# rainfall1998/3D_reconstruction_system

Hardware: AMD Instinct MI355X
Metric: Mpoints/s fused (1280x384 depth, N frames) (higher is better)
Workload: dtype f64; 1 GPU; C2: 1280x384 u8 depth x 100 frames per GPU -> float32 xyz, fused unproject+SE(3); every step reads the NEXT of 16 resident rasters (786 MB, beyond the 256 MiB Infinity Cache): fresh inputs from HBM, staged by the library's sweep, as in a pipeline that touches every frame once; inputs=fresh, frames_per_gpu=100, step=1 fused launch over this rank's frames (shards stay resident), assemble=none, assemble_choice=auto, parallelism=frames sharded, 1 rank(s), one process per GPU

## Files before the change

### 3d_reconstruction_system_amd/csrc/r3d_fuse.hip

```cpp
#include <algorithm>
#include <cstdlib>
#include <type_traits>

#include "r3d_internal.h"
#include "r3d_magic_div.h"
#include "r3d_voxel_dev.h"

namespace {

constexpr int kThreads = 256;
constexpr int kPx = 4;
constexpr int kTile = kThreads * kPx;
constexpr int kStageChunkMB = 96;

struct FuseDims {
  double scale;
  uint32_t hw;
  uint32_t width;
  uint32_t tiles_per_frame;
  uint32_t n_frames;
  uint32_t w_magic;
  uint32_t w_shift;
  uint32_t t_magic;
  uint32_t t_shift;
  uint32_t total_tiles;
  uint32_t rgb_vec_ok;
  uint32_t depth_vec_ok;
};

using r3d_magic::magic_div;
using r3d_magic::make_magic;

struct Pose {
  double r[9];
  double t[3];
};

template <bool POSE>
__device__ __forceinline__ void load_pose(const double* __restrict__ pose, uint32_t frame, Pose& P) {
  if (POSE) {
    const double* pp = pose + (uint64_t)frame * 12;
#pragma unroll
    for (int k = 0; k < 9; ++k) P.r[k] = pp[k];
#pragma unroll
    for (int k = 0; k < 3; ++k) P.t[k] = pp[9 + k];
  }
}

template <bool POSE>
__device__ __forceinline__ void point(double z, double u, double v, const Pose& p, double o[3]) {
  const double x = u * z;
  const double y = v * z;
  if (POSE) {
    const double dx = x - p.t[0], dy = y - p.t[1], dz = z - p.t[2];
    o[0] = fma(p.r[2], dz, fma(p.r[1], dy, p.r[0] * dx));
    o[1] = fma(p.r[5], dz, fma(p.r[4], dy, p.r[3] * dx));
    o[2] = fma(p.r[8], dz, fma(p.r[7], dy, p.r[6] * dx));
  } else {
    o[0] = x;
    o[1] = y;
    o[2] = z;
  }
}

typedef float f32x3 __attribute__((ext_vector_type(3)));
typedef uint32_t u32x4 __attribute__((ext_vector_type(4)));
typedef uint32_t u32x3 __attribute__((ext_vector_type(3)));

__device__ __forceinline__ void store_x3_nt(void* dst, f32x3 v) {
  asm volatile("global_store_dwordx3 %0, %1, off nt\n\ts_nop 1" ::"v"(dst), "v"(v) : "memory");
}
__device__ __forceinline__ void store_x3_nt(void* dst, u32x3 v) {
  asm volatile("global_store_dwordx3 %0, %1, off nt\n\ts_nop 1" ::"v"(dst), "v"(v) : "memory");
}

template <typename DT, int ITEMS, int SHIFT, bool CLAMP>
__device__ __forceinline__ void load_tile(const DT* __restrict__ depth, const FuseDims& dm, uint32_t tile, uint32_t tid,
                                          DT raw[ITEMS]) {
  const uint32_t frame = magic_div(tile, dm.t_magic, dm.t_shift);
  const uint32_t tf = tile - frame * dm.tiles_per_frame;
  const uint64_t fbase = (uint64_t)frame * dm.hw;
#pragma unroll
  for (int r = 0; r < ITEMS; ++r) {
    const uint32_t p = tf * kTile + ((r * kThreads + tid) >> SHIFT);
    if (CLAMP)
      raw[r] = depth[fbase + min(p, dm.hw - 1)];
    else
      raw[r] = p < dm.hw ? depth[fbase + p] : DT(0);
  }
}

template <int ROUNDS>
__device__ __forceinline__ void load_tile_wave(const uint8_t* __restrict__ depth, const FuseDims& dm, uint64_t fbase, uint32_t tf,
                                               uint32_t tid, uint8_t raw[ROUNDS]) {
  const uint32_t lane = tid & 63u, wave = tid >> 6;
  const bool whole = dm.depth_vec_ok && (tf + 1) * kTile <= dm.hw;
  if (whole) {
    const uint32_t dw = reinterpret_cast<const uint32_t*>(depth + fbase + (uint64_t)tf * kTile)[tid];
#pragma unroll
    for (int r = 0; r < ROUNDS; ++r) {
      const uint32_t got = (uint32_t)__builtin_amdgcn_ds_bpermute((int)((16u * r + (lane >> 2)) << 2), (int)dw);
      raw[r] = (uint8_t)(got >> (8u * (lane & 3u)));
    }
  } else {
#pragma unroll
    for (int r = 0; r < ROUNDS; ++r) {
      const uint32_t p = tf * kTile + 256u * wave + 64u * r + lane;
      raw[r] = depth[fbase + min(p, dm.hw - 1)];
    }
  }
}

struct StageSlices {
  const uint4* src;
  uint64_t n16;
  uint32_t n_stage;
};

__device__ __forceinline__ uint32_t touch_pieces(const uint4* __restrict__ src, uint64_t lo, uint64_t hi) {
  uint32_t acc = 0;
  for (uint64_t base = lo + threadIdx.x; base < hi; base += kThreads * 4) {
    uint4 q[4];
#pragma unroll
    for (int k = 0; k < 4; ++k) {
      const uint64_t i = base + (uint64_t)k * kThreads;
      q[k] = src[i < hi ? i : hi - 1];
    }
#pragma unroll
    for (int k = 0; k < 4; ++k) acc ^= q[k].x ^ q[k].y ^ q[k].z ^ q[k].w;
  }
  return acc;
}

template <bool POSE, bool RAGGED>
__device__ __forceinline__ void store_tile(float* __restrict__ out, const FuseDims& dm, const Pose& P, uint64_t fbase,
                                           const uint32_t p[kPx], const double z[kPx], const double ui[kPx],
                                           const double vj[kPx]) {
#pragma unroll
  for (int r = 0; r < kPx; ++r) {
    double w[3];
    point<POSE>(z[r], ui[r], vj[r], P, w);
    if (!RAGGED || p[r] < dm.hw) store_x3_nt(out + (fbase + p[r]) * 3, f32x3{(float)w[0], (float)w[1], (float)w[2]});
  }
}

template <typename DT, bool POSE, bool WAVE>
__global__ __launch_bounds__(kThreads) void fuse_lane_kernel(const DT* __restrict__ depth, float* __restrict__ out,
                                                             const double* __restrict__ u, const double* __restrict__ v,
                                                             const double* __restrict__ pose, const FuseDims dm,
                                                             const StageSlices st) {
  if (blockIdx.x < st.n_stage) {
    const uint64_t lo = st.n16 * blockIdx.x / st.n_stage, hi = st.n16 * (blockIdx.x + 1) / st.n_stage;
    const uint32_t acc = touch_pieces(st.src, lo, hi);
    if (acc == 0x9e3779b9u && st.n16 == ~(uint64_t)0) out[0] = (float)acc;
    return;
  }
  const uint32_t tid = threadIdx.x;
  const uint32_t first = WAVE ? 256u * (tid >> 6) + (tid & 63u) : tid;
  constexpr uint32_t kRound = WAVE ? 64u : (uint32_t)kThreads;
  for (uint32_t tile = blockIdx.x - st.n_stage; tile < dm.total_tiles; tile += gridDim.x - st.n_stage) {
    const uint32_t frame = magic_div(tile, dm.t_magic, dm.t_shift);
    const uint32_t tf = tile - frame * dm.tiles_per_frame;
    Pose P;
    load_pose<POSE>(pose, frame, P);
    const uint64_t fbase = (uint64_t)frame * dm.hw;
    const uint32_t t0 = tf * kTile;
    DT raw[kPx];
    if constexpr (WAVE)
      load_tile_wave<kPx>(depth, dm, fbase, tf, tid, raw);
    else
      load_tile<DT, kPx, 0, true>(depth, dm, tile, tid, raw);
    uint32_t p[kPx];
    double z[kPx], ui[kPx], vj[kPx];
#pragma unroll
    for (int r = 0; r < kPx; ++r) {
      p[r] = t0 + r * kRound + first;
      const uint32_t pc = min(p[r], dm.hw - 1);
      const uint32_t j = magic_div(pc, dm.w_magic, dm.w_shift);
      ui[r] = u[pc - j * dm.width];
      vj[r] = v[j];
    }
    __builtin_amdgcn_s_waitcnt(0);
#pragma unroll
    for (int r = 0; r < kPx; ++r) z[r] = (double)raw[r] * dm.scale;
    if (t0 + kTile <= dm.hw)
      store_tile<POSE, false>(out, dm, P, fbase, p, z, ui, vj);
    else
      store_tile<POSE, true>(out, dm, P, fbase, p, z, ui, vj);
  }
}

template <typename DT, bool POSE>
__global__ __launch_bounds__(kThreads) void fuse_pair_kernel(const DT* __restrict__ depth, double* __restrict__ out,
                                                             const double* __restrict__ u, const double* __restrict__ v,
                                                             const double* __restrict__ pose, const FuseDims dm) {
  constexpr int kItems = 2 * kPx;
  const uint32_t tid = threadIdx.x;
  const bool odd = tid & 1u;
  for (uint32_t tile = blockIdx.x; tile < dm.total_tiles; tile += gridDim.x) {
    const uint32_t frame = magic_div(tile, dm.t_magic, dm.t_shift);
    const uint32_t tf = tile - frame * dm.tiles_per_frame;
    Pose P;
    load_pose<POSE>(pose, frame, P);
    double ra[3], rb[3];
    if (POSE) {
#pragma unroll
      for (int c = 0; c < 3; ++c) {
        ra[c] = odd ? P.r[3 + c] : P.r[c];
        rb[c] = odd ? P.r[6 + c] : P.r[3 + c];
      }
    }
    const uint64_t fbase = (uint64_t)frame * dm.hw;
    DT raw[kItems];
    load_tile<DT, kItems, 1, (sizeof(DT) > 1)>(depth, dm, tile, tid, raw);
    uint32_t* tile_out = reinterpret_cast<uint32_t*>(out) + (fbase + (uint64_t)tf * kTile) * 6;
#pragma unroll
    for (int r = 0; r < kItems; ++r) {
      const uint32_t q = r * kThreads + tid;
      const uint32_t p = tf * kTile + (q >> 1);
      if (p < dm.hw) {
        const uint32_t j = magic_div(p, dm.w_magic, dm.w_shift);
        const uint32_t i = p - j * dm.width;
        const double z = (double)raw[r] * dm.scale;
        const double x = u[i] * z;
        const double y = v[j] * z;
        double a, b;
        if (POSE) {
          const double dx = x - P.t[0], dy = y - P.t[1], dz = z - P.t[2];
          a = fma(ra[2], dz, fma(ra[1], dy, ra[0] * dx));
          b = fma(rb[2], dz, fma(rb[1], dy, rb[0] * dx));
        } else {
          a = odd ? y : x;
          b = odd ? z : y;
        }
        const uint32_t alo = (uint32_t)__double2loint(a), ahi = (uint32_t)__double2hiint(a);
        const uint32_t blo = (uint32_t)__double2loint(b), bhi = (uint32_t)__double2hiint(b);
        store_x3_nt(tile_out + (uint64_t)q * 3, odd ? u32x3{ahi, blo, bhi} : u32x3{alo, ahi, blo});
      }
    }
  }
}

template <typename DT, bool POSE>
__global__ __launch_bounds__(kThreads) void fuse_rgb_kernel(const DT* __restrict__ depth, const uint8_t* __restrict__ rgb,
                                                            float* __restrict__ out, uint32_t* __restrict__ rgba_out,
                                                            const double* __restrict__ u, const double* __restrict__ v,
                                                            const double* __restrict__ pose, const FuseDims dm) {
  __shared__ __attribute__((aligned(16))) uint8_t lds[kTile * 3];
  const uint32_t tid = threadIdx.x;
  auto is_staged = [&](uint32_t tile) {
    const uint32_t frame = magic_div(tile, dm.t_magic, dm.t_shift);
    const uint32_t tf = tile - frame * dm.tiles_per_frame;
    return dm.rgb_vec_ok && (tf + 1) * kTile <= dm.hw;
  };
  auto colour_chunk = [&](uint32_t tile) -> u32x4 {
    const uint32_t frame = magic_div(tile, dm.t_magic, dm.t_shift);
    const uint32_t tf = tile - frame * dm.tiles_per_frame;
    return reinterpret_cast<const u32x4*>(rgb + ((uint64_t)frame * dm.hw + (uint64_t)tf * kTile) * 3)[tid];
  };
  for (uint32_t tile = blockIdx.x; tile < dm.total_tiles; tile += gridDim.x) {
    const uint32_t frame = magic_div(tile, dm.t_magic, dm.t_shift);
    const uint32_t tf = tile - frame * dm.tiles_per_frame;
    Pose P;
    load_pose<POSE>(pose, frame, P);
    const uint64_t fbase = (uint64_t)frame * dm.hw;
    const bool staged = is_staged(tile);
    DT raw[kPx];
    u32x4 ccur = {0, 0, 0, 0};
    load_tile<DT, kPx, 0, true>(depth, dm, tile, tid, raw);
    if (staged && tid < kTile * 3 / 16) ccur = colour_chunk(tile);
    if (staged) {
      if (tid < kTile * 3 / 16) reinterpret_cast<u32x4*>(lds)[tid] = ccur;
      __syncthreads();
    }
#pragma unroll
    for (int r = 0; r < kPx; ++r) {
      const uint32_t l = r * kThreads + tid;
      const uint32_t p = tf * kTile + l;
      if (p < dm.hw) {
        const uint32_t j = magic_div(p, dm.w_magic, dm.w_shift);
        const uint32_t i = p - j * dm.width;
        double w[3];
        point<POSE>((double)raw[r] * dm.scale, u[i], v[j], P, w);
        store_x3_nt(out + (fbase + p) * 3, f32x3{(float)w[0], (float)w[1], (float)w[2]});
        uint32_t c;
        if (staged) {
          c = (uint32_t)lds[l * 3] | ((uint32_t)lds[l * 3 + 1] << 8) | ((uint32_t)lds[l * 3 + 2] << 16);
        } else {
          const uint8_t* s = rgb + (fbase + p) * 3;
          c = (uint32_t)s[0] | ((uint32_t)s[1] << 8) | ((uint32_t)s[2] << 16);
        }
        __builtin_nontemporal_store(c, rgba_out + fbase + p);
      }
    }
    if (staged) __syncthreads();
  }
}

constexpr uint64_t kVoxelRun = 64;

struct VoxelView {
  uint64_t* table;
  unsigned long long* counters;
  double factor;
  int log2cap;
};

template <typename DT, bool POSE, bool RGB>
__global__ __launch_bounds__(kThreads) void fuse_voxel_kernel(const DT* __restrict__ depth, const uint8_t* __restrict__ rgb,
                                                              float* __restrict__ out, uint32_t* __restrict__ rgba_out,
                                                              const double* __restrict__ u, const double* __restrict__ v,
                                                              const double* __restrict__ pose, const FuseDims dm,
                                                              const VoxelView vv) {
  using namespace r3d_vox;
  __shared__ __attribute__((aligned(16))) uint8_t lds[RGB ? kTile * 3 : 16];
  __shared__ unsigned long long local_set[kLdsSlots];
  __shared__ unsigned local_fill[3];
  const uint32_t tid = threadIdx.x;
  const int lane = tid & 63;
  const uint64_t mask = ((uint64_t)1 << vv.log2cap) - 1;
  unsigned n_new = 0, n_ignored = 0, n_over = 0;
  const uint32_t per_wg = (dm.total_tiles + gridDim.x - 1) / gridDim.x;
  const uint64_t lo64 = (uint64_t)blockIdx.x * per_wg;
  const uint32_t tile_lo = lo64 < dm.total_tiles ? (uint32_t)lo64 : dm.total_tiles;
  const uint32_t tile_hi = dm.total_tiles - tile_lo < per_wg ? dm.total_tiles : tile_lo + per_wg;
  for (int k = tid; k < kLdsSlots; k += kThreads) local_set[k] = kEmpty;
  if (tid < 3) local_fill[tid] = 0;
  auto flush = [&]() {
#pragma unroll
    for (int k = 0; k < kLdsSlots / kThreads; ++k) {
      const int s = k * kThreads + tid;
      const uint64_t code = local_set[s];
      if (code != kEmpty) {
        local_set[s] = kEmpty;
        const int r = table_insert(vv.table, mask, vv.log2cap, code);
        n_new += r > 0 ? 1u : 0u;
        n_over += r < 0 ? 1u : 0u;
      }
    }
  };
  unsigned total = 0, j = 0;
  for (uint32_t tile = tile_lo; tile < tile_hi; ++tile, ++j) {
    lds_settle();
    __syncthreads();
    if (j > 0) total += local_fill[(j - 1) % 3];
    if (tid == 0) local_fill[(j + 1) % 3] = 0;
    if (total >= (unsigned)kLdsKeepBelow) {
      flush();
      total = 0;
    }
    const uint32_t frame = magic_div(tile, dm.t_magic, dm.t_shift);
    const uint32_t tf = tile - frame * dm.tiles_per_frame;
    Pose P;
    load_pose<POSE>(pose, frame, P);
    const uint64_t fbase = (uint64_t)frame * dm.hw;
    const bool staged = RGB && dm.rgb_vec_ok && (tf + 1) * kTile <= dm.hw;
    DT raw[kPx];
    load_tile<DT, kPx, 0, true>(depth, dm, tile, tid, raw);
    if (RGB && staged && tid < kTile * 3 / 16)
      reinterpret_cast<u32x4*>(lds)[tid] = reinterpret_cast<const u32x4*>(rgb + (fbase + (uint64_t)tf * kTile) * 3)[tid];
    lds_settle();
    __syncthreads();
    unsigned claimed = 0;
#pragma unroll
    for (int r = 0; r < kPx; ++r) {
      const uint32_t l = r * kThreads + tid;
      const uint32_t p = tf * kTile + l;
      uint64_t code = kEmpty;
      bool live = p < dm.hw;
      if (live) {
        const uint32_t jrow = magic_div(p, dm.w_magic, dm.w_shift);
        const uint32_t i = p - jrow * dm.width;
        double w[3];
        point<POSE>((double)raw[r] * dm.scale, u[i], v[jrow], P, w);
        const float fx = (float)w[0], fy = (float)w[1], fz = (float)w[2];
        store_x3_nt(out + (fbase + p) * 3, f32x3{fx, fy, fz});
        if (RGB) {
          uint32_t c;
          if (staged) {
            c = (uint32_t)lds[l * 3] | ((uint32_t)lds[l * 3 + 1] << 8) | ((uint32_t)lds[l * 3 + 2] << 16);
          } else {
            const uint8_t* sp = rgb + (fbase + p) * 3;
            c = (uint32_t)sp[0] | ((uint32_t)sp[1] << 8) | ((uint32_t)sp[2] << 16);
          }
          __builtin_nontemporal_store(c, rgba_out + fbase + p);
        }
        if (!voxel_key(fx, fy, fz, vv.factor, &code)) {
          ++n_ignored;
          live = false;
          code = kEmpty;
        }
      }
      const uint64_t prev = prev_lane_u64(code);
      if (live && lane > 0 && prev == code) live = false;
      if (live) {
        bool mine = false;
        const bool done = lds_set_claim(local_set, code, &mine);
        claimed += mine ? 1u : 0u;
        if (!done) {
          const int r2 = table_insert(vv.table, mask, vv.log2cap, code);
          n_new += r2 > 0 ? 1u : 0u;
          n_over += r2 < 0 ? 1u : 0u;
        }
      }
    }
#pragma unroll
    for (int off = 32; off > 0; off >>= 1) claimed += __shfl_down(claimed, off, 64);
    if (lane == 0 && claimed) atomicAdd(&local_fill[j % 3], claimed);
  }
  __syncthreads();
  flush();
  const auto [w_new, w_ignored, w_over] = r3d_vox::wave_sum(n_new, n_ignored, n_over);
  if (lane == 0) {
    if (w_new) atomicAdd(&vv.counters[0], (unsigned long long)w_new);
    if (w_ignored) atomicAdd(&vv.counters[1], (unsigned long long)w_ignored);
    if (w_over) atomicAdd(&vv.counters[2], (unsigned long long)w_over);
  }
}

__global__ __launch_bounds__(kThreads) void rgb_expand_kernel(const uint8_t* __restrict__ rgb, uint32_t* __restrict__ rgba_out,
                                                              uint64_t n, uint32_t vec_ok) {
  __shared__ __attribute__((aligned(16))) uint8_t lds[kTile * 3];
  const uint32_t tid = threadIdx.x;
  const uint64_t n_tiles = (n + kTile - 1) / kTile;
  for (uint64_t tile = blockIdx.x; tile < n_tiles; tile += gridDim.x) {
    const uint64_t base = tile * kTile;
    const bool staged = vec_ok && base + kTile <= n;
    if (staged) {
      if (tid < kTile * 3 / 16) reinterpret_cast<uint4*>(lds)[tid] = reinterpret_cast<const uint4*>(rgb + base * 3)[tid];
      __syncthreads();
    }
#pragma unroll
    for (int r = 0; r < kPx; ++r) {
      const uint32_t l = r * kThreads + tid;
      if (base + l < n) {
        uint32_t c;
        if (staged) {
          c = (uint32_t)lds[l * 3] | ((uint32_t)lds[l * 3 + 1] << 8) | ((uint32_t)lds[l * 3 + 2] << 16);
        } else {
          const uint8_t* s = rgb + (base + l) * 3;
          c = (uint32_t)s[0] | ((uint32_t)s[1] << 8) | ((uint32_t)s[2] << 16);
        }
        __builtin_nontemporal_store(c, rgba_out + base + l);
      }
    }
    if (staged) __syncthreads();
  }
}

__global__ __launch_bounds__(kThreads) void cache_touch_kernel(const uint4* __restrict__ src, uint64_t n16,
                                                               uint32_t* __restrict__ sink) {
  uint32_t acc = 0;
  const uint64_t stride = (uint64_t)gridDim.x * (kThreads * 4);
  for (uint64_t base = (uint64_t)blockIdx.x * (kThreads * 4) + threadIdx.x; base < n16; base += stride) {
    uint4 q[4];
#pragma unroll
    for (int k = 0; k < 4; ++k) {
      const uint64_t i = base + (uint64_t)k * kThreads;
      q[k] = src[i < n16 ? i : n16 - 1];
    }
#pragma unroll
    for (int k = 0; k < 4; ++k) acc ^= q[k].x ^ q[k].y ^ q[k].z ^ q[k].w;
  }
  if (acc == 0x9e3779b9u && n16 == ~(uint64_t)0) *sink = acc;
}

StageSlices stage_slices(const r3d_ctx* ctx, const void* p, uint64_t bytes) {
  const uintptr_t lo = ((uintptr_t)p + 15) & ~(uintptr_t)15, hi = ((uintptr_t)p + bytes) & ~(uintptr_t)15;
  if (hi <= lo) return StageSlices{nullptr, 0, 0};
  const uint64_t n16 = (hi - lo) / 16;
  uint64_t blocks = (n16 + kThreads * 4 - 1) / (kThreads * 4);
  if (blocks > (uint64_t)ctx->num_cus * 8) blocks = (uint64_t)ctx->num_cus * 8;
  return StageSlices{reinterpret_cast<const uint4*>(lo), n16, (uint32_t)blocks};
}

void cache_touch(r3d_ctx* ctx, const void* p, uint64_t bytes) {
  const StageSlices st = stage_slices(ctx, p, bytes);
  if (!st.n_stage) return;
  hipLaunchKernelGGL(cache_touch_kernel, dim3(st.n_stage), dim3(kThreads), 0, ctx->stream, st.src, st.n16,
                     static_cast<uint32_t*>(nullptr));
}

struct FusePtrs {
  const void* depth;
  void* out;
  const double* u;
  const double* v;
  const double* pose;
  const uint8_t* rgb;
  uint32_t* rgba;
};

template <typename DT, bool POSE>
void launch_typed(const FusePtrs& p, const FuseDims& dm, int out_dtype, int blocks, bool wave, const StageSlices& st,
                  hipStream_t s) {
  const DT* d = static_cast<const DT*>(p.depth);
  if (out_dtype == R3D_F64) {
    hipLaunchKernelGGL((fuse_pair_kernel<DT, POSE>), dim3(blocks), dim3(kThreads), 0, s, d, static_cast<double*>(p.out), p.u,
                       p.v, p.pose, dm);
  } else if (p.rgb) {
    hipLaunchKernelGGL((fuse_rgb_kernel<DT, POSE>), dim3(blocks), dim3(kThreads), 0, s, d, p.rgb, static_cast<float*>(p.out),
                       p.rgba, p.u, p.v, p.pose, dm);
  } else {
    if constexpr (std::is_same<DT, uint8_t>::value && !POSE) {
      if (wave) {
        hipLaunchKernelGGL((fuse_lane_kernel<DT, POSE, true>), dim3(blocks + st.n_stage), dim3(kThreads), 0, s, d,
                           static_cast<float*>(p.out), p.u, p.v, p.pose, dm, st);
        return;
      }
    }
    hipLaunchKernelGGL((fuse_lane_kernel<DT, POSE, false>), dim3(blocks + st.n_stage), dim3(kThreads), 0, s, d,
                       static_cast<float*>(p.out), p.u, p.v, p.pose, dm, st);
  }
}

template <bool POSE>
void launch_depth(const FusePtrs& p, const FuseDims& dm, int depth_dtype, int out_dtype, int blocks, bool wave,
                  const StageSlices& st, hipStream_t s) {
  switch (depth_dtype) {
    case R3D_DEPTH_U8: launch_typed<uint8_t, POSE>(p, dm, out_dtype, blocks, wave, st, s); break;
    case R3D_DEPTH_U16: launch_typed<uint16_t, POSE>(p, dm, out_dtype, blocks, wave, st, s); break;
    default: launch_typed<float, POSE>(p, dm, out_dtype, blocks, wave, st, s); break;
  }
}

template <typename DT>
void launch_voxel_typed(const FusePtrs& p, const FuseDims& dm, const VoxelView& vv, bool with_pose, int blocks, hipStream_t s) {
  const DT* d = static_cast<const DT*>(p.depth);
  float* o = static_cast<float*>(p.out);
#define R3D_LAUNCH_FV(POSE, RGB)                                                                                         \
  hipLaunchKernelGGL((fuse_voxel_kernel<DT, POSE, RGB>), dim3(blocks), dim3(kThreads), 0, s, d, p.rgb, o, p.rgba, p.u, p.v, \
                     p.pose, dm, vv)
  if (with_pose) {
    if (p.rgb) R3D_LAUNCH_FV(true, true); else R3D_LAUNCH_FV(true, false);
  } else {
    if (p.rgb) R3D_LAUNCH_FV(false, true); else R3D_LAUNCH_FV(false, false);
  }
#undef R3D_LAUNCH_FV
}

void launch_voxel(const FusePtrs& p, const FuseDims& dm, const VoxelView& vv, int depth_dtype, bool with_pose, int blocks,
                  hipStream_t s) {
  switch (depth_dtype) {
    case R3D_DEPTH_U8: launch_voxel_typed<uint8_t>(p, dm, vv, with_pose, blocks, s); break;
    case R3D_DEPTH_U16: launch_voxel_typed<uint16_t>(p, dm, vv, with_pose, blocks, s); break;
    default: launch_voxel_typed<float>(p, dm, vv, with_pose, blocks, s); break;
  }
}

int fuse_common(r3d_ctx* ctx, const r3d_camera* cam, const void* d_depth, int depth_dtype, int n_frames,
                double depth_scale, const double* d_pose, bool with_pose, void* d_out, int out_dtype,
                const uint8_t* d_rgb = nullptr, uint32_t* d_rgba = nullptr, r3d_voxelset* vs = nullptr) {
  int rc = r3d_ctx_enter(ctx);
  if (rc) return rc;
  R3D_REQUIRE(cam != nullptr, "camera is NULL");
  VoxelView vv{nullptr, nullptr, 0.0, 0};
  if (vs) {
    r3d_ctx* vctx = nullptr;
    if ((rc = r3d_voxelset_device_view(vs, &vctx, &vv.factor, &vv.table, &vv.log2cap, &vv.counters))) return rc;
    R3D_REQUIRE(vctx == ctx, "voxel set belongs to a different ctx");
    R3D_REQUIRE(out_dtype == R3D_F32, "the voxel keys are taken from the f32 cloud: out_dtype must be R3D_F32");
  }
  R3D_REQUIRE(cam->ctx == ctx, "camera belongs to a different ctx");
  R3D_REQUIRE(depth_dtype >= R3D_DEPTH_U8 && depth_dtype <= R3D_DEPTH_F32, "unknown depth dtype %d", depth_dtype);
  R3D_REQUIRE(out_dtype == R3D_F32 || out_dtype == R3D_F64, "unknown output dtype %d", out_dtype);
  R3D_REQUIRE(n_frames >= 0, "n_frames must be >= 0");
  R3D_REQUIRE((d_rgb == nullptr) == (d_rgba == nullptr), "colour needs both the rgb plane and the rgba output");
  if (n_frames == 0) return R3D_OK;
  R3D_REQUIRE(d_depth && d_out, "NULL device pointer");
  R3D_REQUIRE(!with_pose || d_pose, "pose table is NULL");
  const uint64_t hw = (uint64_t)cam->height * cam->width;
  const uint64_t dsz = r3d_depth_size(depth_dtype), osz = 3 * (uint64_t)r3d_xyz_size(out_dtype);
  {
    const uint64_t all_tiles = ((hw + kTile - 1) / kTile) * (uint64_t)n_frames;
    R3D_REQUIRE(all_tiles < ((uint64_t)1 << 31), "batch too large for one launch (%llu tiles); split the frames",
                (unsigned long long)all_tiles);
  }
  const bool colour_after = d_rgb && out_dtype == R3D_F64;
  const bool wave = !with_pose && out_dtype == R3D_F32 && depth_dtype == R3D_DEPTH_U8 && !(d_rgb && !colour_after);
  const bool rgb_in_kernel = d_rgb && !colour_after;
  const uint64_t in_per_frame = hw * (dsz + (rgb_in_kernel ? 3 : 0));
  const uint64_t in_bytes = in_per_frame * (uint64_t)n_frames;
  const uint64_t chunk_bytes = (uint64_t)(ctx->fuse_chunk_mb > 0 ? ctx->fuse_chunk_mb : kStageChunkMB) << 20;
  const uint64_t budget = (uint64_t)ctx->fuse_resident_mb << 20;
  const uint64_t depth_bytes = hw * dsz * (uint64_t)n_frames, rgb_bytes = rgb_in_kernel ? hw * 3 * (uint64_t)n_frames : 0;
  const bool small_inputs = dsz <= 2 || (out_dtype == R3D_F64 && !rgb_in_kernel);
  bool stage_depth = ctx->fuse_prefetch == 2, stage_rgb = ctx->fuse_prefetch == 2 && rgb_in_kernel;
  if (ctx->fuse_prefetch == 0 && small_inputs && in_bytes > ((uint64_t)ctx->fuse_stage_auto_mb << 20)) {
    stage_depth = !r3d_inputs_resident(ctx, d_depth, depth_bytes, budget);
    stage_rgb = rgb_in_kernel && !r3d_inputs_resident(ctx, d_rgb, rgb_bytes, budget);
  }
  const bool stage = stage_depth || stage_rgb;
  r3d_wrote(ctx, d_out, hw * osz * (uint64_t)n_frames);
  r3d_inputs_read(ctx, d_depth, depth_bytes, budget);
  if (rgb_in_kernel) r3d_inputs_read(ctx, d_rgb, rgb_bytes, budget);
  int frames_per_step = n_frames;
  if (stage) {
    const uint64_t f = chunk_bytes / (in_per_frame ? in_per_frame : 1);
    frames_per_step = (int)(f < 1 ? 1 : (f > (uint64_t)n_frames ? (uint64_t)n_frames : f));
  }
  for (int f0 = 0; f0 < n_frames; f0 += frames_per_step) {
    const int nf = n_frames - f0 < frames_per_step ? n_frames - f0 : frames_per_step;
    const uint64_t px0 = hw * (uint64_t)f0;
    const char* dd = static_cast<const char*>(d_depth) + px0 * dsz;
    const uint8_t* rr = d_rgb ? d_rgb + px0 * 3 : nullptr;
    FusePtrs p{dd, static_cast<char*>(d_out) + px0 * osz, cam->d_u, cam->d_v, with_pose ? d_pose + (uint64_t)f0 * 12 : nullptr,
               colour_after ? nullptr : rr, d_rgba ? d_rgba + px0 : nullptr};
    FuseDims dm;
    dm.scale = depth_scale;
    dm.hw = (uint32_t)hw;
    dm.width = (uint32_t)cam->width;
    dm.tiles_per_frame = (uint32_t)((hw + kTile - 1) / kTile);
    dm.n_frames = (uint32_t)nf;
    make_magic(dm.width, &dm.w_magic, &dm.w_shift);
    make_magic(dm.tiles_per_frame, &dm.t_magic, &dm.t_shift);
    const uint64_t total_tiles = (uint64_t)dm.tiles_per_frame * nf;
    dm.total_tiles = (uint32_t)total_tiles;
    dm.rgb_vec_ok = rr && ((uintptr_t)rr % 16 == 0) && (hw % 16 == 0);
    dm.depth_vec_ok = ((uintptr_t)dd % 4 == 0) && ((hw * dsz) % 4 == 0);
    const bool fold = stage_depth && ctx->fuse_stage_fold && !vs && out_dtype == R3D_F32 && !p.rgb && total_tiles < (1u << 30);
    StageSlices st{nullptr, 0, 0};
    if (fold)
      st = stage_slices(ctx, dd, hw * dsz * (uint64_t)nf);
    else if (stage_depth)
      cache_touch(ctx, dd, hw * dsz * (uint64_t)nf);
    if (stage_rgb) cache_touch(ctx, rr, hw * 3 * (uint64_t)nf);
    ctx->fuse_sweeps += (int)stage_depth + (int)stage_rgb;
    const bool stride8 = !wave && !with_pose && out_dtype == R3D_F32 && depth_dtype == R3D_DEPTH_U8 && !p.rgb;
    uint64_t blocks = ctx->fuse_blocks > 0 ? (uint64_t)ctx->fuse_blocks : stride8 ? (uint64_t)ctx->num_cus * 8 : total_tiles;
    if (blocks > total_tiles) blocks = total_tiles;
    if (vs) {
      uint64_t g = ctx->fuse_blocks > 0 ? (uint64_t)ctx->fuse_blocks
                                         : std::max<uint64_t>((uint64_t)ctx->num_cus * 8, (total_tiles + kVoxelRun - 1) / kVoxelRun);
      if (g > total_tiles) g = total_tiles;
      launch_voxel(p, dm, vv, depth_dtype, with_pose, (int)g, ctx->stream);
    } else if (with_pose)
      launch_depth<true>(p, dm, depth_dtype, out_dtype, (int)blocks, wave, st, ctx->stream);
    else
      launch_depth<false>(p, dm, depth_dtype, out_dtype, (int)blocks, wave, st, ctx->stream);
  }
  if (colour_after) {
    const uint64_t n = hw * (uint64_t)n_frames;
    uint64_t b = (n + kTile - 1) / kTile;
    if (b > (uint64_t)ctx->num_cus * 16) b = (uint64_t)ctx->num_cus * 16;
    hipLaunchKernelGGL(rgb_expand_kernel, dim3((unsigned)b), dim3(kThreads), 0, ctx->stream, d_rgb, d_rgba, n,
                       (uint32_t)((uintptr_t)d_rgb % 16 == 0));
  }
  R3D_HIP(hipGetLastError());
  return R3D_OK;
}

int fuse_host_common(r3d_ctx* ctx, const r3d_camera* cam, const void* h_depth, int depth_dtype, int n_frames,
                     double depth_scale, const double* h_pose, bool with_pose, void* h_out, int out_dtype) {
  int rc = r3d_ctx_enter(ctx);
  if (rc) return rc;
  R3D_REQUIRE(cam != nullptr, "camera is NULL");
  R3D_REQUIRE(depth_dtype >= R3D_DEPTH_U8 && depth_dtype <= R3D_DEPTH_F32, "unknown depth dtype %d", depth_dtype);
  R3D_REQUIRE(out_dtype == R3D_F32 || out_dtype == R3D_F64, "unknown output dtype %d", out_dtype);
  R3D_REQUIRE(n_frames >= 0, "n_frames must be >= 0");
  if (n_frames == 0) return R3D_OK;
  R3D_REQUIRE(h_depth && h_out, "NULL host pointer");
  R3D_REQUIRE(!with_pose || h_pose, "pose table is NULL");
  const size_t n = (size_t)cam->height * cam->width * n_frames;
  const size_t in_bytes = n * r3d_depth_size(depth_dtype);
  const size_t out_bytes = n * 3 * r3d_xyz_size(out_dtype);
  void *d_in = nullptr, *d_out = nullptr, *d_pose = nullptr;
  if ((rc = r3d_scratch(ctx, 0, in_bytes, &d_in))) return rc;
  if ((rc = r3d_scratch(ctx, 1, out_bytes, &d_out))) return rc;
  if (with_pose) {
    if ((rc = r3d_scratch(ctx, 2, (size_t)n_frames * 12 * sizeof(double), &d_pose))) return rc;
    R3D_HIP(hipMemcpyAsync(d_pose, h_pose, (size_t)n_frames * 12 * sizeof(double), hipMemcpyHostToDevice, ctx->stream));
  }
  const size_t frame_in = (size_t)cam->height * cam->width * r3d_depth_size(depth_dtype);
  const size_t frame_out = (size_t)cam->height * cam->width * 3 * r3d_xyz_size(out_dtype);
  auto launch = [&](int64_t lo, int64_t n) -> int {
    return fuse_common(ctx, cam, static_cast<char*>(d_in) + (size_t)lo * frame_in, depth_dtype, (int)n, depth_scale,
                       with_pose ? static_cast<const double*>(d_pose) + (size_t)lo * 12 : nullptr, with_pose,
                       static_cast<char*>(d_out) + (size_t)lo * frame_out, out_dtype);
  };
  return r3d_host_pipeline(ctx, n_frames, frame_in, frame_out, h_depth, h_out, d_in, d_out, launch);
}

int fuse_rgb_host(r3d_ctx* ctx, const r3d_camera* cam, const void* h_depth, int depth_dtype, int n_frames, double depth_scale,
                  const double* h_pose, const unsigned char* h_rgb, void* h_xyz_out, int out_dtype, uint32_t* h_rgba_out) {
  int rc = r3d_ctx_enter(ctx);
  if (rc) return rc;
  R3D_REQUIRE(cam != nullptr, "camera is NULL");
  R3D_REQUIRE(depth_dtype >= R3D_DEPTH_U8 && depth_dtype <= R3D_DEPTH_F32, "unknown depth dtype %d", depth_dtype);
  R3D_REQUIRE(out_dtype == R3D_F32 || out_dtype == R3D_F64, "unknown output dtype %d", out_dtype);
  R3D_REQUIRE(n_frames >= 0, "n_frames must be >= 0");
  if (n_frames == 0) return R3D_OK;
  R3D_REQUIRE(h_depth && h_rgb && h_xyz_out && h_rgba_out, "NULL host pointer");
  const size_t px = (size_t)cam->height * cam->width, n = px * n_frames;
  const size_t f_depth = px * r3d_depth_size(depth_dtype), f_rgb = px * 3, f_xyz = px * 3 * r3d_xyz_size(out_dtype),
               f_rgba = px * 4;
  void *d_depth = nullptr, *d_xyz = nullptr, *d_pose = nullptr, *d_rgb = nullptr, *d_rgba = nullptr;
  if ((rc = r3d_scratch(ctx, 0, n * r3d_depth_size(depth_dtype), &d_depth))) return rc;
  if ((rc = r3d_scratch(ctx, 1, n * 3 * r3d_xyz_size(out_dtype), &d_xyz))) return rc;
  if ((rc = r3d_scratch(ctx, 3, n * 3, &d_rgb))) return rc;
  if ((rc = r3d_scratch(ctx, 4, n * 4, &d_rgba))) return rc;
  if (h_pose) {
    if ((rc = r3d_scratch(ctx, 2, (size_t)n_frames * 12 * sizeof(double), &d_pose))) return rc;
    R3D_HIP(hipMemcpyAsync(d_pose, h_pose, (size_t)n_frames * 12 * sizeof(double), hipMemcpyHostToDevice, ctx->stream));
  }
  const r3d_pipe_buf ins[2] = {{const_cast<void*>(h_depth), d_depth, f_depth}, {const_cast<unsigned char*>(h_rgb), d_rgb, f_rgb}};
  const r3d_pipe_buf outs[2] = {{h_xyz_out, d_xyz, f_xyz}, {h_rgba_out, d_rgba, f_rgba}};
  auto launch = [&](int64_t lo, int64_t cnt) -> int {
    return fuse_common(ctx, cam, static_cast<char*>(d_depth) + (size_t)lo * f_depth, depth_dtype, (int)cnt, depth_scale,
                       h_pose ? static_cast<const double*>(d_pose) + (size_t)lo * 12 : nullptr, h_pose != nullptr,
                       static_cast<char*>(d_xyz) + (size_t)lo * f_xyz, out_dtype,
                       static_cast<const uint8_t*>(d_rgb) + (size_t)lo * f_rgb, static_cast<uint32_t*>(d_rgba) + (size_t)lo * px);
  };
  return r3d_host_pipeline_multi(ctx, n_frames, ins, 2, outs, 2, launch);
}

}

extern "C" {

int r3d_selftest_magic_div(uint32_t d, uint32_t x, uint32_t* q_out) {
  if (d == 0 || x >= ((uint32_t)1 << 31) || !q_out) {
    r3d_set_error("r3d_selftest_magic_div: d must be >= 1, x < 2^31");
    return R3D_ERR_INVALID;
  }
  uint32_t m = 0, sh = 0;
  make_magic(d, &m, &sh);
  *q_out = (uint32_t)(((uint64_t)x * m) >> sh);
  return R3D_OK;
}

int r3d_cache_prefetch(r3d_ctx* ctx, const void* d_ptr, size_t bytes) {
  int rc = r3d_ctx_enter(ctx);
  if (rc) return rc;
  if (bytes == 0) return R3D_OK;
  R3D_REQUIRE(d_ptr != nullptr, "NULL device pointer");
  cache_touch(ctx, d_ptr, bytes);
  r3d_inputs_read(ctx, d_ptr, bytes, (size_t)ctx->fuse_resident_mb << 20);
  R3D_HIP(hipGetLastError());
  return R3D_OK;
}

int r3d_unproject(r3d_ctx* ctx, const r3d_camera* cam, const void* d_depth, int depth_dtype, int n_frames,
                  double depth_scale, void* d_xyz_out, int out_dtype) {
  return fuse_common(ctx, cam, d_depth, depth_dtype, n_frames, depth_scale, nullptr, false, d_xyz_out, out_dtype);
}

int r3d_unproject_host(r3d_ctx* ctx, const r3d_camera* cam, const void* h_depth, int depth_dtype, int n_frames,
                       double depth_scale, void* h_xyz_out, int out_dtype) {
  return fuse_host_common(ctx, cam, h_depth, depth_dtype, n_frames, depth_scale, nullptr, false, h_xyz_out,
                          out_dtype);
}

int r3d_fuse_frames(r3d_ctx* ctx, const r3d_camera* cam, const void* d_depth, int depth_dtype, int n_frames,
                    double depth_scale, const double* d_pose, void* d_xyz_out, int out_dtype) {
  return fuse_common(ctx, cam, d_depth, depth_dtype, n_frames, depth_scale, d_pose, true, d_xyz_out, out_dtype);
}

int r3d_fuse_frames_host(r3d_ctx* ctx, const r3d_camera* cam, const void* h_depth, int depth_dtype, int n_frames,
                         double depth_scale, const double* h_pose, void* h_xyz_out, int out_dtype) {
  return fuse_host_common(ctx, cam, h_depth, depth_dtype, n_frames, depth_scale, h_pose, true, h_xyz_out,
                          out_dtype);
}

int r3d_fuse_frames_rgb(r3d_ctx* ctx, const r3d_camera* cam, const void* d_depth, int depth_dtype, int n_frames,
                        double depth_scale, const double* d_pose, const unsigned char* d_rgb, void* d_xyz_out,
                        int out_dtype, uint32_t* d_rgba_out) {
  R3D_REQUIRE(n_frames == 0 || (d_rgb && d_rgba_out), "colour plane / rgba output is NULL");
  return fuse_common(ctx, cam, d_depth, depth_dtype, n_frames, depth_scale, d_pose, d_pose != nullptr, d_xyz_out, out_dtype,
                     d_rgb, d_rgba_out);
}

int r3d_fuse_frames_voxel(r3d_ctx* ctx, const r3d_camera* cam, const void* d_depth, int depth_dtype, int n_frames,
                          double depth_scale, const double* d_pose, const unsigned char* d_rgb, float* d_xyz_out,
                          uint32_t* d_rgba_out, r3d_voxelset* vs) {
  R3D_REQUIRE(vs != nullptr, "voxel set is NULL");
  R3D_REQUIRE((d_rgb == nullptr) == (d_rgba_out == nullptr), "colour needs both the rgb plane and the rgba output");
  R3D_REQUIRE(ctx != nullptr && cam != nullptr, "NULL argument");
  {
    r3d_ctx* vctx = nullptr;
    VoxelView view;
    int rc = r3d_voxelset_device_view(vs, &vctx, &view.factor, &view.table, &view.log2cap, &view.counters);
    if (rc) return rc;
    R3D_REQUIRE(vctx == ctx, "voxel set belongs to a different ctx");
  }
  const bool with_pose = d_pose != nullptr;
  const int64_t hw = (int64_t)cam->height * cam->width, total = hw * (int64_t)n_frames;
  const int path = ctx->voxel_path;
  if (path == 1 || n_frames <= 0 || !r3d_voxelset_sort_feasible(vs, total, path == 2)) {
    if (n_frames > 0) ctx->voxel_last_path = 1;
    return fuse_common(ctx, cam, d_depth, depth_dtype, n_frames, depth_scale, d_pose, with_pose, d_xyz_out, R3D_F32, d_rgb,
                       d_rgba_out, vs);
  }
  const int64_t want = (int64_t)1 << 18;
  const int f0 = path == 2 ? n_frames : (int)std::min<int64_t>(n_frames, std::max<int64_t>(1, (want + hw - 1) / hw));
  int rc = fuse_common(ctx, cam, d_depth, depth_dtype, f0, depth_scale, d_pose, with_pose, d_xyz_out, R3D_F32, d_rgb, d_rgba_out);
  if (rc) return rc;
  bool sort = path == 2;
  if (!sort && (rc = r3d_voxelset_sample(vs, d_xyz_out, hw * f0, total, 1.5, &sort))) return rc;
  const size_t dsz = r3d_depth_size(depth_dtype);
  const char* depth_rest = static_cast<const char*>(d_depth) + (size_t)hw * f0 * dsz;
  const double* pose_rest = with_pose ? d_pose + (size_t)f0 * 12 : nullptr;
  const unsigned char* rgb_rest = d_rgb ? d_rgb + (size_t)hw * f0 * 3 : nullptr;
  uint32_t* rgba_rest = d_rgba_out ? d_rgba_out + (size_t)hw * f0 : nullptr;
  float* xyz_rest = d_xyz_out + (size_t)hw * f0 * 3;
  if (sort) {
    if (f0 < n_frames && (rc = fuse_common(ctx, cam, depth_rest, depth_dtype, n_frames - f0, depth_scale, pose_rest, with_pose, xyz_rest,
                                           R3D_F32, rgb_rest, rgba_rest)))
      return rc;
    return r3d_voxelset_insert_path(vs, d_xyz_out, total, 2);
  }
  if ((rc = r3d_voxelset_insert_path(vs, d_xyz_out, hw * f0, 1))) return rc;
  if (f0 == n_frames) return R3D_OK;
  return fuse_common(ctx, cam, depth_rest, depth_dtype, n_frames - f0, depth_scale, pose_rest, with_pose, xyz_rest, R3D_F32, rgb_rest,
                     rgba_rest, vs);
}

int r3d_fuse_frames_rgb_host(r3d_ctx* ctx, const r3d_camera* cam, const void* h_depth, int depth_dtype, int n_frames,
                             double depth_scale, const double* h_pose, const unsigned char* h_rgb, void* h_xyz_out,
                             int out_dtype, uint32_t* h_rgba_out) {
  return fuse_rgb_host(ctx, cam, h_depth, depth_dtype, n_frames, depth_scale, h_pose, h_rgb, h_xyz_out, out_dtype, h_rgba_out);
}

}
```

Before: 506,800 Mpoints/s.

## Fold cache staging sweep into f64, RGB and voxel fuse kernels

Extends the in-kernel staging prologue, where extra leading workgroups touch the depth/colour input, from the f32 depth kernel to the f64 pair, RGB and voxel kernels. This replaces a separate cache_touch launch, and a new helper splits a capped staging-workgroup budget between the depth and colour sweeps. The f64 pair kernel also gets an occupancy hint in its launch bounds. This removes a launch and serialisation, but staging blocks now compete with the fuse blocks for bandwidth and CUs.

Result: no change. 507,000 Mpoints/s, median of 3 (+0.0%).

```diff
diff --git a/3d_reconstruction_system_amd/csrc/r3d_fuse.hip b/3d_reconstruction_system_amd/csrc/r3d_fuse.hip
--- a/3d_reconstruction_system_amd/csrc/r3d_fuse.hip
+++ b/3d_reconstruction_system_amd/csrc/r3d_fuse.hip
@@ -132,6 +132,26 @@
   return acc;
 }
 
+__device__ __forceinline__ void stage_slice(const StageSlices& st, uint32_t wg, void* sink) {
+  const uint64_t lo = st.n16 * wg / st.n_stage, hi = st.n16 * (wg + 1) / st.n_stage;
+  const uint32_t acc = touch_pieces(st.src, lo, hi);
+  if (acc == 0x9e3779b9u && st.n16 == ~(uint64_t)0) *static_cast<uint32_t*>(sink) = acc;
+}
+
+__device__ __forceinline__ bool stage_prologue(const StageSlices& st, void* sink) {
+  if (blockIdx.x >= st.n_stage) return false;
+  stage_slice(st, blockIdx.x, sink);
+  return true;
+}
+
+__device__ __forceinline__ bool stage_prologue(const StageSlices& sd, const StageSlices& sc, void* sink) {
+  if (blockIdx.x >= sd.n_stage + sc.n_stage) return false;
+  const bool first = blockIdx.x < sd.n_stage;
+  const StageSlices st{first ? sd.src : sc.src, first ? sd.n16 : sc.n16, first ? sd.n_stage : sc.n_stage};
+  stage_slice(st, first ? blockIdx.x : blockIdx.x - sd.n_stage, sink);
+  return true;
+}
+
 template <bool POSE, bool RAGGED>
 __device__ __forceinline__ void store_tile(float* __restrict__ out, const FuseDims& dm, const Pose& P, uint64_t fbase,
                                            const uint32_t p[kPx], const double z[kPx], const double ui[kPx],
@@ -149,12 +169,7 @@
                                                              const double* __restrict__ u, const double* __restrict__ v,
                                                              const double* __restrict__ pose, const FuseDims dm,
                                                              const StageSlices st) {
-  if (blockIdx.x < st.n_stage) {
-    const uint64_t lo = st.n16 * blockIdx.x / st.n_stage, hi = st.n16 * (blockIdx.x + 1) / st.n_stage;
-    const uint32_t acc = touch_pieces(st.src, lo, hi);
-    if (acc == 0x9e3779b9u && st.n16 == ~(uint64_t)0) out[0] = (float)acc;
-    return;
-  }
+  if (stage_prologue(st, out)) return;
   const uint32_t tid = threadIdx.x;
   const uint32_t first = WAVE ? 256u * (tid >> 6) + (tid & 63u) : tid;
   constexpr uint32_t kRound = WAVE ? 64u : (uint32_t)kThreads;
@@ -191,13 +206,15 @@
 }
 
 template <typename DT, bool POSE>
-__global__ __launch_bounds__(kThreads) void fuse_pair_kernel(const DT* __restrict__ depth, double* __restrict__ out,
+__global__ __launch_bounds__(kThreads, 8) void fuse_pair_kernel(const DT* __restrict__ depth, double* __restrict__ out,
                                                              const double* __restrict__ u, const double* __restrict__ v,
-                                                             const double* __restrict__ pose, const FuseDims dm) {
+                                                             const double* __restrict__ pose, const FuseDims dm,
+                                                             const StageSlices st) {
+  if (stage_prologue(st, out)) return;
   constexpr int kItems = 2 * kPx;
   const uint32_t tid = threadIdx.x;
   const bool odd = tid & 1u;
-  for (uint32_t tile = blockIdx.x; tile < dm.total_tiles; tile += gridDim.x) {
+  for (uint32_t tile = blockIdx.x - st.n_stage; tile < dm.total_tiles; tile += gridDim.x - st.n_stage) {
     const uint32_t frame = magic_div(tile, dm.t_magic, dm.t_shift);
     const uint32_t tf = tile - frame * dm.tiles_per_frame;
     Pose P;
@@ -245,8 +262,11 @@
 __global__ __launch_bounds__(kThreads) void fuse_rgb_kernel(const DT* __restrict__ depth, const uint8_t* __restrict__ rgb,
                                                             float* __restrict__ out, uint32_t* __restrict__ rgba_out,
                                                             const double* __restrict__ u, const double* __restrict__ v,
-                                                            const double* __restrict__ pose, const FuseDims dm) {
+                                                            const double* __restrict__ pose, const FuseDims dm,
+                                                            const StageSlices sd, const StageSlices sc) {
   __shared__ __attribute__((aligned(16))) uint8_t lds[kTile * 3];
+  if (stage_prologue(sd, sc, out)) return;
+  const uint32_t n_stage = sd.n_stage + sc.n_stage;
   const uint32_t tid = threadIdx.x;
   auto is_staged = [&](uint32_t tile) {
     const uint32_t frame = magic_div(tile, dm.t_magic, dm.t_shift);
@@ -258,7 +278,7 @@
     const uint32_t tf = tile - frame * dm.tiles_per_frame;
     return reinterpret_cast<const u32x4*>(rgb + ((uint64_t)frame * dm.hw + (uint64_t)tf * kTile) * 3)[tid];
   };
-  for (uint32_t tile = blockIdx.x; tile < dm.total_tiles; tile += gridDim.x) {
+  for (uint32_t tile = blockIdx.x - n_stage; tile < dm.total_tiles; tile += gridDim.x - n_stage) {
     const uint32_t frame = magic_div(tile, dm.t_magic, dm.t_shift);
     const uint32_t tf = tile - frame * dm.tiles_per_frame;
     Pose P;
@@ -311,17 +331,19 @@
                                                               float* __restrict__ out, uint32_t* __restrict__ rgba_out,
                                                               const double* __restrict__ u, const double* __restrict__ v,
                                                               const double* __restrict__ pose, const FuseDims dm,
-                                                              const VoxelView vv) {
+                                                              const VoxelView vv, const StageSlices sd, const StageSlices sc) {
   using namespace r3d_vox;
   __shared__ __attribute__((aligned(16))) uint8_t lds[RGB ? kTile * 3 : 16];
   __shared__ unsigned long long local_set[kLdsSlots];
   __shared__ unsigned local_fill[3];
+  if (stage_prologue(sd, sc, out)) return;
+  const uint32_t n_fuse = gridDim.x - (sd.n_stage + sc.n_stage), wg = blockIdx.x - (sd.n_stage + sc.n_stage);
   const uint32_t tid = threadIdx.x;
   const int lane = tid & 63;
   const uint64_t mask = ((uint64_t)1 << vv.log2cap) - 1;
   unsigned n_new = 0, n_ignored = 0, n_over = 0;
-  const uint32_t per_wg = (dm.total_tiles + gridDim.x - 1) / gridDim.x;
-  const uint64_t lo64 = (uint64_t)blockIdx.x * per_wg;
+  const uint32_t per_wg = (dm.total_tiles + n_fuse - 1) / n_fuse;
+  const uint64_t lo64 = (uint64_t)wg * per_wg;
   const uint32_t tile_lo = lo64 < dm.total_tiles ? (uint32_t)lo64 : dm.total_tiles;
   const uint32_t tile_hi = dm.total_tiles - tile_lo < per_wg ? dm.total_tiles : tile_lo + per_wg;
   for (int k = tid; k < kLdsSlots; k += kThreads) local_set[k] = kEmpty;
@@ -474,6 +496,15 @@
   return StageSlices{reinterpret_cast<const uint4*>(lo), n16, (uint32_t)blocks};
 }
 
+void stage_share(const r3d_ctx* ctx, StageSlices& a, StageSlices& b) {
+  const uint64_t cap = (uint64_t)ctx->num_cus * 8;
+  if (!a.n_stage || !b.n_stage || (uint64_t)a.n_stage + b.n_stage <= cap) return;
+  uint64_t na = (uint64_t)((double)cap * (double)a.n16 / ((double)a.n16 + (double)b.n16) + 0.5);
+  na = std::min<uint64_t>(std::max<uint64_t>(na, 1), cap - 1);
+  a.n_stage = (uint32_t)std::min<uint64_t>(na, a.n_stage);
+  b.n_stage = (uint32_t)std::min<uint64_t>(cap - na, b.n_stage);
+}
+
 void cache_touch(r3d_ctx* ctx, const void* p, uint64_t bytes) {
   const StageSlices st = stage_slices(ctx, p, bytes);
   if (!st.n_stage) return;
@@ -493,14 +524,14 @@
 
 template <typename DT, bool POSE>
 void launch_typed(const FusePtrs& p, const FuseDims& dm, int out_dtype, int blocks, bool wave, const StageSlices& st,
-                  hipStream_t s) {
+                  const StageSlices& sc, hipStream_t s) {
   const DT* d = static_cast<const DT*>(p.depth);
   if (out_dtype == R3D_F64) {
-    hipLaunchKernelGGL((fuse_pair_kernel<DT, POSE>), dim3(blocks), dim3(kThreads), 0, s, d, static_cast<double*>(p.out), p.u,
-                       p.v, p.pose, dm);
+    hipLaunchKernelGGL((fuse_pair_kernel<DT, POSE>), dim3(blocks + st.n_stage), dim3(kThreads), 0, s, d,
+                       static_cast<double*>(p.out), p.u, p.v, p.pose, dm, st);
   } else if (p.rgb) {
-    hipLaunchKernelGGL((fuse_rgb_kernel<DT, POSE>), dim3(blocks), dim3(kThreads), 0, s, d, p.rgb, static_cast<float*>(p.out),
-                       p.rgba, p.u, p.v, p.pose, dm);
+    hipLaunchKernelGGL((fuse_rgb_kernel<DT, POSE>), dim3(blocks + st.n_stage + sc.n_stage), dim3(kThreads), 0, s, d, p.rgb,
+                       static_cast<float*>(p.out), p.rgba, p.u, p.v, p.pose, dm, st, sc);
   } else {
     if constexpr (std::is_same<DT, uint8_t>::value && !POSE) {
       if (wave) {
@@ -516,21 +547,22 @@
 
 template <bool POSE>
 void launch_depth(const FusePtrs& p, const FuseDims& dm, int depth_dtype, int out_dtype, int blocks, bool wave,
-                  const StageSlices& st, hipStream_t s) {
+                  const StageSlices& st, const StageSlices& sc, hipStream_t s) {
   switch (depth_dtype) {
-    case R3D_DEPTH_U8: launch_typed<uint8_t, POSE>(p, dm, out_dtype, blocks, wave, st, s); break;
-    case R3D_DEPTH_U16: launch_typed<uint16_t, POSE>(p, dm, out_dtype, blocks, wave, st, s); break;
-    default: launch_typed<float, POSE>(p, dm, out_dtype, blocks, wave, st, s); break;
+    case R3D_DEPTH_U8: launch_typed<uint8_t, POSE>(p, dm, out_dtype, blocks, wave, st, sc, s); break;
+    case R3D_DEPTH_U16: launch_typed<uint16_t, POSE>(p, dm, out_dtype, blocks, wave, st, sc, s); break;
+    default: launch_typed<float, POSE>(p, dm, out_dtype, blocks, wave, st, sc, s); break;
   }
 }
 
 template <typename DT>
-void launch_voxel_typed(const FusePtrs& p, const FuseDims& dm, const VoxelView& vv, bool with_pose, int blocks, hipStream_t s) {
+void launch_voxel_typed(const FusePtrs& p, const FuseDims& dm, const VoxelView& vv, bool with_pose, int blocks,
+                        const StageSlices& st, const StageSlices& sc, hipStream_t s) {
   const DT* d = static_cast<const DT*>(p.depth);
   float* o = static_cast<float*>(p.out);
-#define R3D_LAUNCH_FV(POSE, RGB)                                                                                         \
-  hipLaunchKernelGGL((fuse_voxel_kernel<DT, POSE, RGB>), dim3(blocks), dim3(kThreads), 0, s, d, p.rgb, o, p.rgba, p.u, p.v, \
-                     p.pose, dm, vv)
+#define R3D_LAUNCH_FV(POSE, RGB)                                                                                            \
+  hipLaunchKernelGGL((fuse_voxel_kernel<DT, POSE, RGB>), dim3(blocks + st.n_stage + sc.n_stage), dim3(kThreads), 0, s, d, p.rgb, \
+                     o, p.rgba, p.u, p.v, p.pose, dm, vv, st, sc)
   if (with_pose) {
     if (p.rgb) R3D_LAUNCH_FV(true, true); else R3D_LAUNCH_FV(true, false);
   } else {
@@ -540,11 +572,11 @@
 }
 
 void launch_voxel(const FusePtrs& p, const FuseDims& dm, const VoxelView& vv, int depth_dtype, bool with_pose, int blocks,
-                  hipStream_t s) {
+                  const StageSlices& st, const StageSlices& sc, hipStream_t s) {
   switch (depth_dtype) {
-    case R3D_DEPTH_U8: launch_voxel_typed<uint8_t>(p, dm, vv, with_pose, blocks, s); break;
-    case R3D_DEPTH_U16: launch_voxel_typed<uint16_t>(p, dm, vv, with_pose, blocks, s); break;
-    default: launch_voxel_typed<float>(p, dm, vv, with_pose, blocks, s); break;
+    case R3D_DEPTH_U8: launch_voxel_typed<uint8_t>(p, dm, vv, with_pose, blocks, st, sc, s); break;
+    case R3D_DEPTH_U16: launch_voxel_typed<uint16_t>(p, dm, vv, with_pose, blocks, st, sc, s); break;
+    default: launch_voxel_typed<float>(p, dm, vv, with_pose, blocks, st, sc, s); break;
   }
 }
 
@@ -618,13 +650,16 @@
     dm.total_tiles = (uint32_t)total_tiles;
     dm.rgb_vec_ok = rr && ((uintptr_t)rr % 16 == 0) && (hw % 16 == 0);
     dm.depth_vec_ok = ((uintptr_t)dd % 4 == 0) && ((hw * dsz) % 4 == 0);
-    const bool fold = stage_depth && ctx->fuse_stage_fold && !vs && out_dtype == R3D_F32 && !p.rgb && total_tiles < (1u << 30);
-    StageSlices st{nullptr, 0, 0};
-    if (fold)
-      st = stage_slices(ctx, dd, hw * dsz * (uint64_t)nf);
-    else if (stage_depth)
-      cache_touch(ctx, dd, hw * dsz * (uint64_t)nf);
-    if (stage_rgb) cache_touch(ctx, rr, hw * 3 * (uint64_t)nf);
+    const bool fold = stage && ctx->fuse_stage_fold && total_tiles < (1u << 30);
+    StageSlices st{nullptr, 0, 0}, sc{nullptr, 0, 0};
+    if (fold) {
+      if (stage_depth) st = stage_slices(ctx, dd, hw * dsz * (uint64_t)nf);
+      if (stage_rgb) sc = stage_slices(ctx, rr, hw * 3 * (uint64_t)nf);
+      stage_share(ctx, st, sc);
+    } else {
+      if (stage_depth) cache_touch(ctx, dd, hw * dsz * (uint64_t)nf);
+      if (stage_rgb) cache_touch(ctx, rr, hw * 3 * (uint64_t)nf);
+    }
     ctx->fuse_sweeps += (int)stage_depth + (int)stage_rgb;
     const bool stride8 = !wave && !with_pose && out_dtype == R3D_F32 && depth_dtype == R3D_DEPTH_U8 && !p.rgb;
     uint64_t blocks = ctx->fuse_blocks > 0 ? (uint64_t)ctx->fuse_blocks : stride8 ? (uint64_t)ctx->num_cus * 8 : total_tiles;
@@ -633,11 +668,11 @@
       uint64_t g = ctx->fuse_blocks > 0 ? (uint64_t)ctx->fuse_blocks
                                          : std::max<uint64_t>((uint64_t)ctx->num_cus * 8, (total_tiles + kVoxelRun - 1) / kVoxelRun);
       if (g > total_tiles) g = total_tiles;
-      launch_voxel(p, dm, vv, depth_dtype, with_pose, (int)g, ctx->stream);
+      launch_voxel(p, dm, vv, depth_dtype, with_pose, (int)g, st, sc, ctx->stream);
     } else if (with_pose)
-      launch_depth<true>(p, dm, depth_dtype, out_dtype, (int)blocks, wave, st, ctx->stream);
+      launch_depth<true>(p, dm, depth_dtype, out_dtype, (int)blocks, wave, st, sc, ctx->stream);
     else
-      launch_depth<false>(p, dm, depth_dtype, out_dtype, (int)blocks, wave, st, ctx->stream);
+      launch_depth<false>(p, dm, depth_dtype, out_dtype, (int)blocks, wave, st, sc, ctx->stream);
   }
   if (colour_after) {
     const uint64_t n = hw * (uint64_t)n_frames;
```
